# louissmit/VBNN

Measured on AMD Instinct MI355X. Metric: VBLinear fwd+bwd samples/sec, higher is better.
Workload: dtype bf16; 1 GPU; 784-4096-4096-10 VBLinear MLP, batch 4096 per GPU, LRT, S=1; mode=lrt, global_batch=4096, parallelism=dp1, warmup_steps_run=260, backward_order=every updateGradInput, then the accGradParameters from the first layer up, launch=one stream launch per kernel

## Files before the change

### include/vbnn_hip.h

```cpp
#ifndef VBNN_HIP_H
#define VBNN_HIP_H

#include <stddef.h>
#include <stdint.h>

#ifdef __cplusplus
extern "C" {
#endif
#if defined(__GNUC__)
#pragma GCC visibility push(default)
#endif

#define VBNN_ABI_VERSION 6
#define VBNN_KPAD 64

enum { VBNN_OK = 0, VBNN_ERR_INVALID = 1, VBNN_ERR_HIP = 2, VBNN_ERR_NOMEM = 3, VBNN_ERR_UNSUPPORTED = 4 };
enum { VBNN_F32 = 0, VBNN_BF16 = 1 };
enum { VBNN_PACK_COPY = 0, VBNN_PACK_EXP = 1, VBNN_PACK_SQUARE = 2, VBNN_PACK_MUL = 3,
       VBNN_PACK_RELU = 4, VBNN_PACK_RELU_SQUARE = 5 };

typedef struct vbnn_ctx vbnn_ctx;

int vbnn_abi_version(void);
const char* vbnn_last_error(void);
// ... 110 lines not shown
    void* g_prev; void* gv_prev; int64_t ld_gp;
    void* gT_prev; void* gvT_prev; int64_t ld_gpT;
    const void* w; const void* w2; int64_t ld_w;
} vbnn_dx_args;

int vbnn_grad_input(vbnn_ctx* ctx, int dtype, const vbnn_dx_args* a);

typedef struct vbnn_dw_args {
    const void* xT;
    const void* x2T;
    const void* gT;
    const void* gvT;
    int64_t ld_n;
    int64_t N, I, O;
    float scale;
    int accumulate;
    float* gradWeight;
    float* gradSum;
    uint64_t seed; uint32_t layer; uint32_t draw;
    const float* lvars;
    float* grad_mu; float* grad_lv;
    const float* means; const double* stats; float B; float S; float kl_scale;
    float* gradBias;
    const void* x; const void* x2; const void* g; const void* gv; int64_t ld_x; int64_t ld_g;
    const void* mu_s; const void* var_s; int64_t ld_w;
    int part;
    const uint32_t* draw_dev;
} vbnn_dw_args;

int vbnn_acc_grad_parameters(vbnn_ctx* ctx, int dtype, const vbnn_dw_args* a);

int vbnn_backward_pair(vbnn_ctx* ctx, int dtype, const vbnn_dx_args* dx, const vbnn_dw_args* dw);

int vbnn_acc_grad_bias(vbnn_ctx* ctx, int dtype, const void* g, int64_t ld_g, int64_t N, int64_t O,
                       float scale, int accumulate, float* gradBias);

int vbnn_prep_layer(vbnn_ctx* ctx, int dtype, const float* means, const float* lvars, int64_t O, int64_t I,
                    void* mu_s, void* var_s, int64_t ld_w, void* muT_s, void* varT_s, int64_t ld_wT,
                    double* stats);

typedef struct vbnn_prep_desc {
    const float* means; const float* lvars; int64_t O, I;
    void* mu_s; void* var_s; int64_t ld_w;
    void* muT_s; void* varT_s; int64_t ld_wT;
    double* stats;
} vbnn_prep_desc;
typedef struct vbnn_pack_desc {
    const float* src; int64_t rows, cols, ld_src;
    void* dst; int64_t ld_dst; void* dstT; int64_t ld_dstT;
} vbnn_pack_desc;
int vbnn_prepare(vbnn_ctx* ctx, int dtype, int n_layers, const vbnn_prep_desc* layers, const vbnn_pack_desc* extra);


int vbnn_compute_mugrads(vbnn_ctx* ctx, const float* means, const double* stats, float B, float S,
                         float* gradWeight, float* lcg, int64_t W);
int vbnn_compute_vargrads(vbnn_ctx* ctx, const float* lvars, const float* vars, const float* stdv,
                          const double* stats, float B, float S, float* gradSum, float* lcg, int64_t W);

int vbnn_calc_lc(vbnn_ctx* ctx, const float* means, const float* lvars, const float* vars, const float* mu_sqe,
                 const double* stats, float B, float* lc_elem, double* lc_sum_dev, int64_t W);

int vbnn_pack_input(vbnn_ctx* ctx, int dtype, const float* src, int64_t ld_src, int64_t N, int64_t I, void* x_s,
                    void* x2_s, int64_t ld_x, void* xT_s, void* x2T_s, int64_t ld_xT, int64_t rows_per_draw);


int vbnn_adam_step(vbnn_ctx* ctx, float* x, const float* grad, const float* grad2, float* m, float* v, int64_t n,
// ... 361 lines not shown
```

### vbnn_amd/_lib.py

```python
import ctypes as C
import os
import subprocess

_HERE = os.path.dirname(os.path.abspath(__file__))
LIB_PATH = os.environ.get("VBNN_HIP_LIB") or os.path.join(_HERE, "lib", "libvbnn_hip.so")
CSRC = os.path.join(_HERE, "csrc")

OK = 0
F32, BF16 = 0, 1
PACK_COPY, PACK_EXP, PACK_SQUARE, PACK_MUL, PACK_RELU, PACK_RELU_SQUARE = range(6)
KPAD = 64
STREAM_EPS, STREAM_ZETA, STREAM_INIT, STREAM_DATA, STREAM_HEINIT = 1, 2, 3, 4, 5

_vp, _i64, _u64, _u32, _f, _i = C.c_void_p, C.c_int64, C.c_uint64, C.c_uint32, C.c_float, C.c_int


class VbnnError(RuntimeError):
    pass


class FwdArgs(C.Structure):
    _fields_ = [("w", _vp), ("w2", _vp), ("x", _vp), ("x2", _vp), ("ld_w", _i64), ("ld_x", _i64),
                ("N", _i64), ("I", _i64), ("O", _i64), ("bias", _vp),
                ("seed", _u64), ("layer", _u32), ("draw", _u32), ("row0", _i64),
                ("y", _vp), ("ld_y", _i64), ("r", _vp), ("ld_r", _i64), ("r_packed", _i), ("relu", _i),
                ("h", _vp), ("h2", _vp), ("ld_h", _i64), ("hT", _vp), ("h2T", _vp), ("ld_hT", _i64), ("rows_per_draw", _i64),
                ("draw_dev", _vp), ("head_w3", _vp), ("head_ld_w", _i64), ("head_C", _i64), ("head_slots", _vp)]


class DxArgs(C.Structure):
    _fields_ = [("wT", _vp), ("w2T", _vp), ("g", _vp), ("gv", _vp), ("ld_wT", _i64), ("ld_g", _i64),
                ("N", _i64), ("I", _i64), ("O", _i64), ("x", _vp), ("ld_x", _i64),
                ("gx", _vp), ("ld_gx", _i64), ("relu_mask", _i), ("r_prev", _vp), ("ld_r_prev", _i64), ("r_prev_packed", _i),
                ("g_prev", _vp), ("gv_prev", _vp), ("ld_gp", _i64),
                ("gT_prev", _vp), ("gvT_prev", _vp), ("ld_gpT", _i64),
                ("w", _vp), ("w2", _vp), ("ld_w", _i64)]


class PrepDesc(C.Structure):
    _fields_ = [("means", _vp), ("lvars", _vp), ("O", _i64), ("I", _i64), ("mu_s", _vp), ("var_s", _vp), ("ld_w", _i64),
                ("muT_s", _vp), ("varT_s", _vp), ("ld_wT", _i64), ("stats", _vp)]

# ... 155 lines not shown

_SIGS = {
    "vbnn_abi_version": ([], _i),
    "vbnn_last_error": ([], C.c_char_p),
    "vbnn_debug_set": ([_i, _i], _i),
    "vbnn_debug_get": ([_i], _i),
    "vbnn_kmajor_supported": ([_i64, _i64, _i64], _i),
    "vbnn_kmajor_supported_dw": ([_i64, _i64, _i64, _i], _i),
    "vbnn_ctx_kmajor_supported": ([_vp, _i64, _i64, _i64], _i),
    "vbnn_ctx_kmajor_supported_dw": ([_vp, _i64, _i64, _i64, _i], _i),
    "vbnn_ctx_create": ([_i, _vp, C.POINTER(_vp)], _i),
    "vbnn_ctx_create_cu_budget": ([_i, _i, C.POINTER(_vp)], _i),
    "vbnn_ctx_stream": ([_vp, C.POINTER(_vp), C.POINTER(_i)], _i),
    "vbnn_ctx_destroy": ([_vp], _i),
    "vbnn_ctx_set_stream": ([_vp, _vp], _i),
    "vbnn_sync": ([_vp], _i),
    "vbnn_buf_alloc": ([_vp, C.c_size_t, C.POINTER(_vp)], _i),
    "vbnn_buf_free": ([_vp, _vp], _i),
    "vbnn_buf_zero": ([_vp, _vp, C.c_size_t], _i),
    "vbnn_buf_upload": ([_vp, _vp, _vp, C.c_size_t], _i),
    "vbnn_buf_download": ([_vp, _vp, _vp, C.c_size_t], _i),
    "vbnn_fill_normal": ([_vp, _vp, _i64, _i64, _i64, _u64, _u32, _u32, _u32, _i64, _f], _i),
    "vbnn_fill_normal_hw": ([_vp, _vp, _i64, _i64, _i64, _u64, _u32, _u32, _u32, _i64, _f], _i),
    "vbnn_box_muller_forms": ([_vp, _vp, _vp, _vp, _vp, _i64], _i),
    "vbnn_compute_prior": ([_vp, _vp, _vp, _i64, _vp, _vp, _vp, _vp], _i),
    "vbnn_wn_sample": ([_vp, _vp, _vp, _vp, _vp, _vp, _i64, _i64, _u64, _u32, _u32], _i),
    "vbnn_pack": ([_vp, _i, _i, _vp, _vp, _i64, _i64, _i64, _vp, _i64, _vp, _i64], _i),
    "vbnn_forward": ([_vp, _i, C.POINTER(FwdArgs)], _i),
    "vbnn_forward_head_slots": ([_vp, _i, _i64, _i64, _i64, _i64], _i),
    "vbnn_head_forward_slots": ([_vp, _vp, _i64, _vp, _vp, _i64, _i64, _f, _vp, _vp, _vp, _i, _vp, _vp, _i64], _i),
    "vbnn_grad_input": ([_vp, _i, C.POINTER(DxArgs)], _i),
    "vbnn_acc_grad_parameters": ([_vp, _i, C.POINTER(DwArgs)], _i),
    "vbnn_backward_pair": ([_vp, _i, C.POINTER(DxArgs), C.POINTER(DwArgs)], _i),
    "vbnn_head_forward_backward": ([_vp, _i, C.POINTER(HeadArgs)], _i),
    "vbnn_head_predict": ([_vp, _i, C.POINTER(PredictArgs)], _i),
    "vbnn_predict_moments": ([_vp, C.POINTER(MomentsArgs)], _i),
    "vbnn_acc_grad_bias": ([_vp, _i, _vp, _i64, _i64, _i64, _f, _i, _vp], _i),
    "vbnn_prep_layer": ([_vp, _i, _vp, _vp, _i64, _i64, _vp, _vp, _i64, _vp, _vp, _i64, _vp], _i),
    "vbnn_compute_mugrads": ([_vp, _vp, _vp, _f, _f, _vp, _vp, _i64], _i),
    "vbnn_compute_vargrads": ([_vp, _vp, _vp, _vp, _vp, _f, _f, _vp, _vp, _i64], _i),
    "vbnn_calc_lc": ([_vp, _vp, _vp, _vp, _vp, _vp, _f, _vp, _vp, _i64], _i),
    "vbnn_pack_input": ([_vp, _i, _vp, _i64, _i64, _i64, _vp, _vp, _i64, _vp, _vp, _i64, _i64], _i),
    "vbnn_adam_step": ([_vp, _vp, _vp, _vp, _vp, _vp, _i64, _f, _f, _f, _f, _f, _i64, _vp], _i),
    "vbnn_sgd_step": ([_vp, _vp, _vp, _i64, _f], _i),
    "vbnn_update": ([_vp, _i, _i, _vp, _vp], _i),
    "vbnn_prepare_masked": ([_vp, _i, _i, _vp, _vp, _vp], _i),
    "vbnn_update_masked": ([_vp, _i, _i, _vp, _vp, _vp], _i),
    "vbnn_calc_lc_masked": ([_vp, _vp, _vp, _vp, _vp, _f, _vp, _vp, _i64], _i),
    "vbnn_comm_unique_id": ([_vp], _i),
    "vbnn_comm_create": ([_vp, _i, _i, _vp, C.POINTER(_vp)], _i),
    "vbnn_comm_destroy": ([_vp], _i),
    "vbnn_comm_info": ([_vp, C.POINTER(_i), C.POINTER(_i), C.POINTER(_i)], _i),
    "vbnn_allreduce_grads": ([_vp, _vp, _i64], _i),
    "vbnn_comm_finish": ([_vp], _i),
    "vbnn_allreduce_grads_bf16": ([_vp, _vp, _i64], _i),
    "vbnn_cast_grads": ([_vp, _i, _vp, _vp, _i64], _i),
    "vbnn_comm_allgather_u64": ([_vp, _vp, _vp], _i),
    "vbnn_stats_combine": ([_vp, _i, _i, _vp, _vp], _i),
    "vbnn_transpose_packed": ([_vp, _i, _vp, _i64, _i64, _i64, _vp, _i64], _i),
    "vbnn_comm_reduce_scatter": ([_vp, _vp, _i64], _i),
    "vbnn_comm_all_gather": ([_vp, _vp, _i64], _i),
    "vbnn_p2p_reduce_scatter": ([_vp, C.c_size_t, _i64], _i),
    "vbnn_p2p_all_gather": ([_vp, C.c_size_t, _i64], _i),
    "vbnn_p2p_create": ([_vp, _i, _i, C.c_size_t, C.POINTER(_vp), C.POINTER(_vp), _vp], _i),
    "vbnn_p2p_connect": ([_vp, _vp], _i),
    "vbnn_p2p_allreduce": ([_vp, C.c_size_t, _i64], _i),
# ... 91 lines not shown
```

### vbnn_amd/csrc/gemm.hip

```cpp
#include "gemm_dispatch.h"

extern "C" int vbnn_debug_set(int key, int value) {
    if (key == VBNN_DEBUG_GEMM_KERNEL && value >= 0 && value <= 3) { g_force_kernel = value; return VBNN_OK; }
    if (key == VBNN_DEBUG_V2_SCHEDULE && (value == -1 || value == 0 || value == 2 || value == 4)) { g_v2_sched = value; return VBNN_OK; }
    if (key == VBNN_DEBUG_V2_TILE && (value == 0 || value == 64 || value == 128 || value == 256)) { g_v2_tile = value; return VBNN_OK; }
    if (key == VBNN_DEBUG_V3_MIN_K && value >= 64) { g_v3_min_k = value; return VBNN_OK; }
    if (key == VBNN_DEBUG_V2_PSPLIT && value >= -1 && value <= 1) { g_v2_psplit = value; return VBNN_OK; }
    if (key == VBNN_DEBUG_KMAJOR && value >= 0 && value <= 2) { g_kmajor = value; return VBNN_OK; }
    if (key == VBNN_DEBUG_V3_SPLIT && value >= -1 && value <= 1) { g_v3_split = value; return VBNN_OK; }
    if (key == VBNN_DEBUG_V0 && (value == 0 || value == 1)) { g_v0 = value; return VBNN_OK; }
    if (key == VBNN_DEBUG_HEAD_BACKWARD && value >= -1 && value <= 1) { g_head_stream = value; return VBNN_OK; }
    if (key == VBNN_DEBUG_V3_FOLD_SERIAL && (value == 0 || value == 1)) { g_v3_fold_serial = value; return VBNN_OK; }
    vbnn_set_error("vbnn_debug_set: unknown key %d / value %d", key, value);
    return VBNN_ERR_INVALID;
}
extern "C" int vbnn_debug_get(int key) {
    if (key == VBNN_DEBUG_LAST_HEAD_FORM) return g_last_head_form;
    if (key == VBNN_DEBUG_LAST_GEMM_FORM) return g_last_gemm_form;
    return -1;
}

extern "C" int vbnn_kmajor_supported(int64_t M, int64_t N, int64_t K) { return kmajor_selected(M, N, K) ? 1 : 0; }
extern "C" int vbnn_ctx_kmajor_supported(vbnn_ctx* ctx, int64_t M, int64_t N, int64_t K) {
    vbnn_cu_scope plan(ctx);
    return kmajor_selected(M, N, K) ? 1 : 0;
}
extern "C" int vbnn_kmajor_supported_dw(int64_t I, int64_t O, int64_t N, int bias_row) {
    if (!bias_row && kmajor_selected(I, O, N)) return 1;
    if (I % 4 == 0 && kmajor_dw_v3_split_selected(I + (bias_row ? 1 : 0), O, N)) return 2;
    return kmajor_dw_v2_selected(I + (bias_row ? 1 : 0), O, N) ? 1 : 0;
}
extern "C" int vbnn_ctx_kmajor_supported_dw(vbnn_ctx* ctx, int64_t I, int64_t O, int64_t N, int bias_row) {
    vbnn_cu_scope plan(ctx);
    return vbnn_kmajor_supported_dw(I, O, N, bias_row);
}

extern "C" int vbnn_backward_pair(vbnn_ctx* ctx, int dtype, const vbnn_dx_args* dx, const vbnn_dw_args* dw) {
    VBNN_API_BEGIN
    vbnn_cu_scope plan(ctx);
    int chk = check_dx_args(ctx, dx);
    if (chk != VBNN_OK) return chk;
    chk = check_dw_args(ctx, dtype, dw);
    if (chk != VBNN_OK) return chk;
    VBNN_REQUIRE(dx->N == dw->N && dx->I == dw->I && dx->O == dw->O, "the two argument blocks describe one layer");
    if (dtype == VBNN_F32 && !dx->wT && dx->w && !dw->xT && dw->x && dw->g && dw->part == 0 && g_force_kernel == 0) {
        const bool dual = dx->gv != nullptr;
        const bool dw_dual = dw->gv != nullptr;
        if (dual == dw_dual && (!dual || (dx->w2 && !dw->x2))) {
            const EpiDx<float> ea = make_dx_epi<float>(dx);
            const EpiDw eb = make_dw_epi<float>(dw);
            const int M2 = (int)dw->I + (dw->gradBias ? 1 : 0);
// ... 19 lines not shown
```

### vbnn_amd/csrc/gemm_v3.h

```cpp
#pragma once
#include "gemm_v2.h"

constexpr int V3_BM = 256, V3_BN = 256;
constexpr int V3_APART = 128 * 128;
constexpr int V3_BTILE = 256 * 128;
constexpr int V3_LDS = 4 * V3_APART + 3 * V3_BTILE;

inline int g_v3_min_k = 704;
inline int g_v3_fold_serial = 0;
template <class Epi, class = void> struct v3_fold_pipe { static constexpr int value = 0; };
template <class Epi> struct v3_fold_pipe<Epi, std::void_t<decltype(Epi::FOLD_PIPE)>> { static constexpr int value = Epi::FOLD_PIPE; };

#ifndef V3_ST
#define V3_ST(k) do { } while (0)
#endif


template <bool DUAL, bool AK, bool BK, class Epi, bool SPLIT = false, bool HM = false, int PIPE = v3_fold_pipe<Epi>::value>
__global__ __launch_bounds__(512, 2) void gemm_nt_v3(const bf16_t* __restrict__ A, const bf16_t* __restrict__ A2, int64_t lda,
                                                     const bf16_t* __restrict__ B, const bf16_t* __restrict__ B2, int64_t ldb,
                                                     int M, int N, int nk, int tiles_m, int tiles_n, Epi epi_in) {
    static_assert(!(SPLIT && DUAL), "the split form computes one GEMM of the pair per workgroup");
    static_assert(SPLIT == HM && (!HM || (AK && BK)), "the pair-split launch is the half-height K-major form");
    extern __shared__ __attribute__((aligned(16))) unsigned char lds[];
    V3_ST(0);
    const int tid = threadIdx.x;
    const int lane = tid & 63;
    const int wave = __builtin_amdgcn_readfirstlane(tid >> 6);
    if (wave >= 4) __builtin_amdgcn_s_setprio(1);
    const int wr = wave >> 2, wc = wave & 3;
    Epi epi = epi_in;

    const int nblk = tiles_m * tiles_n * (SPLIT ? 2 : 1);
    int bid = blockIdx.x;
    {
        const int q = nblk >> 3, r = nblk & 7, xcd = bid & 7, idx = bid >> 3;
        bid = (xcd < r ? xcd * (q + 1) : r * (q + 1) + (xcd - r) * q) + idx;
    }
    if (SPLIT) {
        const int ntile = tiles_m * tiles_n;
        const int part = bid / ntile;
        bid -= part * ntile;
        epi.set_part(1 + part);
        if (part) { A = A2; B = B2; }
    }
    int tm, tn;
    {
        constexpr int GM = HM ? 8 : 4, GN = HM ? 4 : 8;
        const int per_band = GM * tiles_n;
        const int band = bid / per_band;
        const int in_band = bid - band * per_band;
        const int band_rows = min(GM, tiles_m - band * GM);
        const int full = band_rows * GN;
        const int grp = in_band / full;
        const int in_grp = in_band - grp * full;
        const int grp_cols = min(GN, tiles_n - grp * GN);
        tm = min(band * GM + in_grp / grp_cols, tiles_m - 1);
        tn = grp * GN + in_grp % grp_cols;
    }
    const int m0 = tm * (HM ? V3_BM / 2 : V3_BM), n0 = tn * V3_BN;

    int a_off[2][2], b_off[4];
    auto hk = [](int kr) { return (kr & 3) | (((kr >> 3) & 1) << 2); };
#pragma unroll
    for (int P = 0; P < 2; ++P)
#pragma unroll
        for (int d = 0; d < 2; ++d) {
// ... 694 lines not shown
                if (DUAL) epi.apply_folded(wm0, wn0 + 4 * p, eln, r1[p], r2[p], pre[b], t1, t2);
                else epi.apply_fast(wm0, wn0 + 4 * p, eln, r1[p], f32x4{0.f, 0.f, 0.f, 0.f}, pre[b], t1, t2);
                if (any_t) {
                    const int nl = 4 * p + q4;
                    const int col = ((nl >> 3) ^ (c16 & 3)) * 8 + (nl & 7);
#pragma unroll
                    for (int j = 0; j < 4; ++j) {
                        tl1[(4 * c16 + j) * TQ + col] = Elt<ET>::to(t1[j]);
                        tl2[(4 * c16 + j) * TQ + col] = Elt<ET>::to(t2[j]);
                    }
                }
                __builtin_amdgcn_sched_barrier(0);
            }
        }
        if (any_t) {
            const int64_t ldt = epi.t_ld();
            const unsigned lo = (unsigned)((lane >> 2) * (int)ldt + 8 * (lane & 3));
#pragma unroll
            for (int pp = 0; pp < 4; ++pp) {
                const int ml = 16 * pp + (lane >> 2);
                const int64_t ub = (int64_t)(wm0 + 16 * pp) * ldt + wn0;
                if (tp1)
                    *reinterpret_cast<bf16x8*>(tp1 + ub + lo) =
                        *reinterpret_cast<const bf16x8*>(tl1 + ml * TQ + 8 * ((lane & 3) ^ ((ml >> 2) & 3)));
                if (tp2)
                    *reinterpret_cast<bf16x8*>(tp2 + ub + lo) =
                        *reinterpret_cast<const bf16x8*>(tl2 + ml * TQ + 8 * ((lane & 3) ^ ((ml >> 2) & 3)));
            }
        }
    });
    V3_ST(4);
}

template <class Epi>
static inline bool gemm_v3_possible(int64_t M, int64_t N, int64_t K, int64_t lda, int64_t ldb, bool ak, bool bk, const Epi& epi) {
    Epi e = epi;
    const bool t_ok = (!e.t1_ptr() && !e.t2_ptr()) ||
                      ((e.t_ld() % 8 == 0) && ((((uintptr_t)e.t1_ptr() | (uintptr_t)e.t2_ptr()) & 15u) == 0));
    const bool a_ok = ak ? (K % V2_BK == 0 && lda % 8 == 0 && lda >= M && K * lda < (1ll << 30)) : M * lda < (1ll << 30);
    const bool b_ok = bk ? (K % V2_BK == 0 && ldb % 8 == 0 && ldb >= N && K * ldb < (1ll << 30)) : N * ldb < (1ll << 30);
    return (M % V3_BM == 0) && (N % V3_BN == 0) && a_ok && b_ok && epi.fast_ok() && epi.v3_ok() && t_ok && M * e.t_ld() < (1ll << 31);
}
static inline bool gemm_v3_shape_ok(int64_t M, int64_t N, int64_t K) {
    if (M % V3_BM || N % V3_BN || K < g_v3_min_k) return false;
    const int64_t cus = vbnn_cu_count();
    const int64_t t3 = (M / V3_BM) * (N / V3_BN), t2 = 2 * t3;
    if (4 * t3 < 3 * cus) return false;
    const int64_t r3 = (t3 + cus - 1) / cus, r2 = (t2 + cus - 1) / cus;
    return 185 * r3 <= 100 * r2;
}
template <class Epi>
static inline bool gemm_v3_eligible(int64_t M, int64_t N, int64_t K, int64_t lda, int64_t ldb, bool ak, bool bk, const Epi& epi) {
    if (!gemm_v3_possible(M, N, K, lda, ldb, ak, bk, epi) || K < g_v3_min_k) return false;
    const int64_t cus = vbnn_cu_count();
    const int64_t t3 = (M / V3_BM) * (N / V3_BN), t2 = 2 * t3;
    if (4 * t3 < 3 * cus) return false;
    const int64_t r3 = (t3 + cus - 1) / cus, r2 = (t2 + cus - 1) / cus;
    return 185 * r3 <= 100 * r2;
}

template <typename T, bool DUAL, bool AK, bool BK, class Epi>
static int launch_gemm_v3(vbnn_ctx* ctx, const T* A, const T* A2, int64_t lda, const T* B, const T* B2, int64_t ldb, int M, int N,
                          int K, const Epi& epi) {
    if constexpr (sizeof(T) != 2) {
        vbnn_set_error("gemm_v3 is bf16 only");
        return VBNN_ERR_UNSUPPORTED;
// ... 4 lines not shown
        }
        const int nk = (K + V2_BK - 1) / V2_BK;
        if ((!AK && lda < (int64_t)nk * V2_BK) || (!BK && ldb < (int64_t)nk * V2_BK)) {
            vbnn_set_error("packed leading dimension too small for K=%d", K);
            return VBNN_ERR_INVALID;
        }
        if (!gemm_v3_possible(M, N, K, lda, ldb, AK, BK, epi)) { vbnn_set_error("gemm_v3: shape / outputs outside its fast path"); return VBNN_ERR_UNSUPPORTED; }
        const int tiles_m = (M + V3_BM - 1) / V3_BM, tiles_n = (N + V3_BN - 1) / V3_BN;
        const void* kern = (const void*)gemm_nt_v3<DUAL, AK, BK, Epi>;
        int form = 0;
        if constexpr (DUAL && v3_fold_pipe<Epi>::value != 0) {
            if (g_v3_fold_serial) { kern = (const void*)gemm_nt_v3<DUAL, AK, BK, Epi, false, false, 0>; form = 1; }
        }
        static vbnn_per_device_flag configured_on[2];
        bool& configured = configured_on[form][ctx->device];
        if (!configured) {
            hipError_t e = hipFuncSetAttribute(kern, hipFuncAttributeMaxDynamicSharedMemorySize, V3_LDS);
            if (e != hipSuccess) { vbnn_set_error("hipFuncSetAttribute: %s", hipGetErrorString(e)); return VBNN_ERR_HIP; }
            configured = true;
        }
        const bf16_t* a = (const bf16_t*)A; const bf16_t* a2 = (const bf16_t*)A2;
        const bf16_t* b = (const bf16_t*)B; const bf16_t* b2 = (const bf16_t*)B2;
        int nk_ = nk, M_ = M, N_ = N, tm_ = tiles_m, tn_ = tiles_n;
        int64_t lda_ = lda, ldb_ = ldb;
        Epi epi_ = epi;
        void* args[] = {&a, &a2, &lda_, &b, &b2, &ldb_, &M_, &N_, &nk_, &tm_, &tn_, &epi_};
        vbnn_note_gemm_form<T>(VBNN_GEMM_KERNEL_V3, 0, 0, DUAL, false, AK, BK, 0, false, form == 1, epi);
        hipError_t e = hipLaunchKernel(kern, dim3(tiles_m * tiles_n), dim3(512), args, V3_LDS, ctx->stream);
        if (e != hipSuccess) { vbnn_set_error("launch of gemm_nt_v3 failed: %s", hipGetErrorString(e)); return VBNN_ERR_HIP; }
        return vbnn_check_launch("gemm_nt_v3");
    }
}

inline int g_v3_split = -1;
static inline bool gemm_v3_split_shape_ok(int64_t M, int64_t N, int64_t K) {
    if (g_v3_split == 0 || N % V3_BN || K % V2_BK) return false;
    if (g_v3_split == 1) return true;
    const int64_t tiles = ((M + V3_BM - 1) / V3_BM) * (N / V3_BN);
    const int64_t blocks = ((M + V3_BM / 2 - 1) / (V3_BM / 2)) * (N / V3_BN) * 2;
    const int64_t cus = vbnn_cu_count();
    return tiles * 16 <= 5 * cus && tiles * 16 >= 3 * cus && K >= 2048 && blocks <= cus && blocks * 8 >= 5 * cus;
}
static inline int64_t gemm_v3_split_lda(int64_t M) { return (M + V3_BM - 1) / V3_BM * V3_BM; }

template <typename T, class Epi>
static int launch_gemm_v3_split(vbnn_ctx* ctx, const T* A, const T* A2, int64_t lda, const T* B, const T* B2, int64_t ldb, int M, int N,
                                int K, const Epi& epi) {
    if constexpr (sizeof(T) != 2 || !Epi::SPLITTABLE || !Epi::EDGE_FAST) {
        return VBNN_ERR_UNSUPPORTED;
    } else {
        Epi e0 = epi;
        if (!A || !A2 || !B || !B2 || !gemm_v3_split_shape_ok(M, N, K) || !epi.fast_ok() || e0.t1_ptr() || e0.t2_ptr() ||
            (((uintptr_t)A | (uintptr_t)B | (uintptr_t)A2 | (uintptr_t)B2) & 15u) != 0 || lda % 8 || ldb % 8 ||
            lda < gemm_v3_split_lda(M) || ldb < N || (int64_t)K * lda >= (1ll << 30) || (int64_t)K * ldb >= (1ll << 30))
            return VBNN_ERR_UNSUPPORTED;
        const int tiles_n = N / V3_BN;
        const int tiles_m = (M + V3_BM / 2 - 1) / (V3_BM / 2);
        const void* kern = (const void*)gemm_nt_v3<false, true, true, Epi, true, true>;
        static vbnn_per_device_flag configured_on;
        bool& configured = configured_on[ctx->device];
        if (!configured) {
            hipError_t e = hipFuncSetAttribute(kern, hipFuncAttributeMaxDynamicSharedMemorySize, V3_LDS);
            if (e != hipSuccess) { vbnn_set_error("hipFuncSetAttribute: %s", hipGetErrorString(e)); return VBNN_ERR_HIP; }
            configured = true;
        }
        const bf16_t* a = (const bf16_t*)A; const bf16_t* a2 = (const bf16_t*)A2;
// ... 12 lines not shown
```

### vbnn_amd/engine.py

```python
import contextlib
import ctypes as C
import math
import os

import torch

from . import _lib as L
from . import partition
from .nn import Context, _DT, _Packed, _VB, _ordered, _p, fill_normal
from .predictive import (LabelPredictResult, PredictResult, QuantilePredictResult, RegressionPredictResult,
                         _Predictive)
from .calibration import CalibrationResult, SelectiveResult, _Calibration
from .pruning import PruneResult, SparsePruneResult, UnitPruneResult, _Pruning
from .checkpoint import CheckpointError, _Checkpoint, digest


_NULL_CM = contextlib.nullcontext()


class _View:

    def __init__(self, t):
        self.t, self.ld = t, t.stride(0)

# ... 40 lines not shown
        ts = self.ctx.torch_stream
        if ts is None:
            return _NULL_CM
        cur = torch.cuda.current_stream(self.device)
        if cur != ts:
            ts.wait_stream(cur)
        return torch.cuda.stream(ts)

    def join(self):
        ts = self.ctx.torch_stream
        if ts is not None:
            cur = torch.cuda.current_stream(self.device)
            if cur != ts:
                cur.wait_stream(ts)

    def _build(self, opt, world_size, rank, process_group, force_reduce):
        self.dtype = opt.get("dtype", "bf16")
        self.code, self.tdt = _DT[self.dtype]
        self.mode = opt.get("mode", "lrt")
        assert self.mode in ("wn", "lrt")
        self.seed = int(opt.get("seed", 3))
        self.world, self.rank, self.pg = world_size, rank, process_group
        self.reduce = world_size > 1 or force_reduce
        self._exchange = None
        self.exchange_dtype = str(opt.get("exchange_dtype", "f32"))
        assert self.exchange_dtype in ("f32", "bf16")
        self._stage, self._staged = None, []
        self.exchange_mode = str(opt.get("exchange_mode", os.environ.get("VBNN_EXCHANGE_MODE", "")) or "allreduce")
        assert self.exchange_mode in ("allreduce", "sharded")
        self.sharded = self.reduce and self.exchange_mode == "sharded"
        self._params_stale = False
        self._dx_first_opt = opt.get("dx_first", None)
        self.fuse_kl = bool(opt.get("fuse_kl", True))
        self.criterion = opt.get("criterion", "nll")
        assert self.criterion in ("nll", "mse", "gauss", "bce")
        self.logvar_clamp = tuple(float(v) for v in opt.get("logvar_clamp", (-20.0, 20.0)))
        if self.criterion == "gauss":
            if int(opt["n_classes"]) % 2:
                raise ValueError(f"criterion = 'gauss': the final Linear holds D means and D log variances (n_classes = "
                                 f"{opt['n_classes']} is odd)")
            if not (len(self.logvar_clamp) == 2 and self.logvar_clamp[0] <= self.logvar_clamp[1]):
                raise ValueError(f"opt.logvar_clamp = {self.logvar_clamp}: (s_min, s_max) with s_min <= s_max")
        self.kl_from_shadows = self.dtype == "bf16" and bool(opt.get("kl_from_shadows", True))
        self.kl_in_update = bool(opt.get("kl_in_update", self.kl_from_shadows and self.fuse_kl and self.mode == "lrt"))
        if self.sharded:
            assert self.fuse_kl and self.mode == "lrt" and self.exchange_dtype == "f32" and not opt.get("overlap", False), \
                "exchange_mode = sharded: the fused LRT engine, fp32 sums, one compute stream"
            assert self.dtype == "bf16" and self.kl_from_shadows, "exchange_mode = sharded: the bf16 configuration (operand shadows)"
            self.kl_in_update = True
        assert not self.kl_in_update or (self.fuse_kl and self.mode == "lrt"), "kl_in_update: the fused LRT engine"
        self.overlap = bool(opt.get("overlap", False))
        self.head_step = bool(opt.get("head_step", True))
        if self.overlap:
            self._side = torch.cuda.Stream(device=self.device)
            self.ctx2 = Context(self.device.index or 0, stream=self._side)
        self.B, self.S = float(opt.get("B", 1e6)), float(opt.get("S", 1))
        hidden = list(opt["hidden"])
        sizes = [opt["input_size"]] + hidden
        self.n_classes = opt["n_classes"]
        self.sizes = sizes
        weights = [sizes[i] * sizes[i + 1] for i in range(len(sizes) - 1)]
        self.dx_first = bool(self._dx_first_opt) if self._dx_first_opt is not None else (2 * min(weights) <= max(weights))
        dev = self.device
        f32 = dict(dtype=torch.float32, device=dev)
        el = opt.get("early_lv", None)
        if el is None:
            el = [(world_size > 1 or force_reduce) and self.mode == "lrt" and bool(opt.get("fuse_kl", True)) and
                  sizes[i] * sizes[i + 1] >= (1 << 22) for i in range(len(hidden))]
        elif isinstance(el, bool):
            el = [el and self.mode == "lrt"] * len(hidden)
        self.early_lv = list(el)
        lay, fin, n_g, self._bucket_ranges = partition.arena_layout(sizes, self.n_classes, self.early_lv)
        self._lay = lay
        self.exchange_kind = str(opt.get("exchange", os.environ.get("VBNN_EXCHANGE", "")) or "")
        n_layers = len(hidden)
        self._plan = partition.sharded_plan(lay, world_size) if self.sharded else None
        arena_extra = None
        if self.reduce and self.exchange_kind == "p2p":
            assert self.exchange_dtype == "f32", "the p2p exchange sums fp32 arenas"
            from .comm import P2PExchange
            n_arena = (n_g + 3) // 4 * 4
            if self.sharded:
                n_arena += sum(2 * _Packed.floats(sizes[i + 1], sizes[i], self.tdt) for i in range(n_layers)) + 8 * world_size * n_layers
            self._exchange = P2PExchange(self.ctx, rank, world_size, n_arena, process_group)
            self.grads = self._exchange.arena[:n_g]
            arena_extra = self._exchange.arena[(n_g + 3) // 4 * 4:]
        else:
            self.grads = torch.zeros(n_g, **f32)

        def carve(n_floats):
            nonlocal arena_extra
            if arena_extra is None:
                return None
            piece, arena_extra = arena_extra[:n_floats], arena_extra[n_floats:]
            return piece
# ... 193 lines not shown

    def _w3_pack_desc(self):
        return L.PackDesc(src=_p(self.weight3), rows=self.n_classes, cols=self.sizes[-1], ld_src=self.sizes[-1],
                          dst=self.w3_s.ptr, ld_dst=self.w3_s.ld, dstT=self.w3T_s.ptr, ld_dstT=self.w3T_s.ld)

    def _lrt(self):
        return self.mode == "lrt" and not self._map

    probe = None

    def _probed(self, name, li):
        if self.probe is None or (self.probe[0] != li and self.probe[0] != "all"):
            return contextlib.nullcontext()
        if self.probe[0] == "all":
            name = f"{name}[{li}]"
        eng = self

        class _Bracket:
            def __enter__(self_inner):
                self_inner.e0 = torch.cuda.Event(enable_timing=True)
                self_inner.e1 = torch.cuda.Event(enable_timing=True)
                self_inner.e0.record()

            def __exit__(self_inner, *exc):
                self_inner.e1.record()
                eng.probe[1].setdefault(name, []).append((self_inner.e0, self_inner.e1))
                return False
        return _Bracket()

    def _probed_part(self, name, li):
        if self.probe is None or self.probe[0] != "all" or not self._early(self.vb[li], self._lrt()):
            return _NULL_CM
        return self._probed(name, li)

    @_ordered
    def clamp_to_map(self):
        self._map = True
        if self.mode == "wn":
            lib = L.lib()
            for v in self.vb:
                L.check(lib.vbnn_pack(self.ctx.h, self.code, L.PACK_COPY, _p(v.means), None, v.I, v.O, v.I,
                                      v.mu_s.ptr, v.mu_s.ld, v.muT_s.ptr if v.muT_s else None,
                                      v.muT_s.ld if v.muT_s else 0))

    def test(self, inputs, targets):
        N = inputs.shape[0]
        self.prepare()
        draws = 1 if self.opt.get("quicktest") else int(self.opt["testSamples"])
        err = acc = 0.0
        for _ in range(draws):
            self._first = True
            if self.opt.get("quicktest"):
                self.clamp_to_map()
            else:
                self.sample()
            self.run(inputs, targets, backward=False)
            loss, correct = self.loss_and_accuracy()
            err += loss * self.world
            acc += 100.0 * correct / (N * (self.n_classes if self.criterion == "bce" else 1))
        return err / draws, acc / draws

    @_ordered
    def sample(self, by=1):
        self.draw += by
        self._map = False
        if self.device_draw:
# ... 214 lines not shown
                                                        inv_n, _p(self.logits), _p(self.out), _p(self.g_logits), accumulate,
                                                        _p(self._acc), _p(self._corr), self._rpd))
                else:
                    L.check(lib.vbnn_head_forward(ctx, code, self.h_s.ptr, self.h_s.ld, self.w3_s.ptr, self.w3_s.ld,
                                                  _p(self.bias3), _p(targets), N, H, Cn, inv_n, _p(self.logits), _p(self.out),
                                                  _p(self.g_logits), accumulate, _p(self._acc), _p(self._corr), self._rpd))
                if not backward:
                    self._first = False
                    return
                L.check(lib.vbnn_head_backward(ctx, code, self.h_s.ptr, self.h_s.ld, self.w3_s.ptr, self.w3_s.ld,
                                               _p(self.g_logits), N, H, Cn, accumulate, _p(self.gradWeight3),
                                               _p(self.gradBias3), _p(vl.gradBias), 1, _p(vl.r) if lrt else None, vl.O, 1,
                                               vl.g_s.ptr,
                                               vl.gv_s.ptr if lrt else None, vl.g_s.ld, vl.gT_s.ptr if vl.gT_s else None,
                                               vl.gvT_s.ptr if (lrt and vl.gvT_s) else None, vl.gT_s.ld if vl.gT_s else 0))
        else:
            if self._rpd:
                targets = targets.repeat(self._draws) if targets.dim() == 1 else targets.repeat(self._draws, 1)
            self._generic_head(N, targets, inv_n, accumulate, backward)
            if not backward:
                self._first = False
                return
        if self.f32_direct and not self.overlap:
            for li in range(nl - 1, -1, -1):
                v = self.vb[li]
                d = self._dw_args(li, N, accumulate)
                with self._probed("accGradParameters", li):
                    if li > 0:
                        L.check(lib.vbnn_backward_pair(ctx, code, C.byref(self._dx_args(li, N)), C.byref(d)))
                    else:
                        L.check(lib.vbnn_acc_grad_parameters(ctx, code, C.byref(d)))
                if not (fused_head and li == nl - 1) and not v.bias_from_dw:
                    L.check(lib.vbnn_acc_grad_bias(ctx, code, v.g_s.ptr, v.g_s.ld, N, v.O, 1.0, accumulate, _p(v.gradBias)))
        elif self.dx_first and not self.reduce and not self.overlap:
            for li in range(nl - 1, 0, -1):
                with self._probed("updateGradInput", li):
                    L.check(lib.vbnn_grad_input(ctx, code, C.byref(self._dx_args(li, N))))
            for li in range(nl):
                v = self.vb[li]
                d = self._dw_args(li, N, accumulate)
                with self._probed("accGradParameters", li):
                    L.check(lib.vbnn_acc_grad_parameters(ctx, code, C.byref(d)))
                if not (fused_head and li == nl - 1) and not v.bias_from_dw:
                    L.check(lib.vbnn_acc_grad_bias(ctx, code, v.g_s.ptr, v.g_s.ld, N, v.O, 1.0, accumulate, _p(v.gradBias)))
        elif not self.overlap:
            for li in range(nl - 1, -1, -1):
                v = self.vb[li]
                d = self._dw_args(li, N, accumulate)
                with self._probed("accGradParameters", li):
                    if self._early(v, lrt):
                        d.part = 2
                        with self._probed_part("accGradParameters.lv", li):
                            L.check(lib.vbnn_acc_grad_parameters(ctx, code, C.byref(d)))
                        if self.sharded:
                            self._scatter(li, ("lv",))
                        else:
                            self._reduce(v.msg_early)
                        d.part = 1
                    with self._probed_part("accGradParameters.mu", li):
                        L.check(lib.vbnn_acc_grad_parameters(ctx, code, C.byref(d)))
                if not (fused_head and li == nl - 1) and not v.bias_from_dw:
                    L.check(lib.vbnn_acc_grad_bias(ctx, code, v.g_s.ptr, v.g_s.ld, N, v.O, 1.0, accumulate, _p(v.gradBias)))
                if self.sharded:
                    self._scatter(li, ("mu", "small") if self._early(v, lrt) else ("lv", "mu", "small"))
                else:
                    self._reduce(v.msg_late if self._early(v, lrt) else (self.bucket_tail if li == nl - 1 else v.bucket))
# ... 306 lines not shown
```

Baseline: 5.572 million samples/s.

## Chain each layer's grad-input and grad-weight GEMMs into one persistent launch

Adds a combined kernel that runs the dX GEMM and the dW GEMM of one hidden layer inside a single launch. Each workgroup computes its tile of the first GEMM, passes an LDS barrier, then computes its tile of the second. The engine enables this by default for bf16 when the dx-first heuristic holds. This reorders the backward pass to per-layer dx/dw pairs. The aim is to cut one kernel launch per layer and the idle tail between the two GEMMs. The cost is a grid sized to the larger of the two GEMMs and a fused kernel that may use registers differently.

```diff
diff --git a/include/vbnn_hip.h b/include/vbnn_hip.h
--- a/include/vbnn_hip.h
+++ b/include/vbnn_hip.h
@@ -166,6 +166,12 @@
 
 int vbnn_backward_pair(vbnn_ctx* ctx, int dtype, const vbnn_dx_args* dx, const vbnn_dw_args* dw);
 
+#define VBNN_CHAIN_DX_FIRST 0
+#define VBNN_CHAIN_DW_FIRST 1
+#define VBNN_DEBUG_LAST_CHAINED 15
+#define VBNN_DEBUG_CHAIN_OFF 16
+int vbnn_backward_chain(vbnn_ctx* ctx, int dtype, const vbnn_dx_args* dx, const vbnn_dw_args* dw, int order);
+
 int vbnn_acc_grad_bias(vbnn_ctx* ctx, int dtype, const void* g, int64_t ld_g, int64_t N, int64_t O,
                        float scale, int accumulate, float* gradBias);
 
diff --git a/vbnn_amd/_lib.py b/vbnn_amd/_lib.py
--- a/vbnn_amd/_lib.py
+++ b/vbnn_amd/_lib.py
@@ -8,6 +8,8 @@
 
 OK = 0
 F32, BF16 = 0, 1
+CHAIN_DX_FIRST, CHAIN_DW_FIRST = 0, 1
+DEBUG_LAST_CHAINED, DEBUG_CHAIN_OFF = 15, 16
 PACK_COPY, PACK_EXP, PACK_SQUARE, PACK_MUL, PACK_RELU, PACK_RELU_SQUARE = range(6)
 KPAD = 64
 STREAM_EPS, STREAM_ZETA, STREAM_INIT, STREAM_DATA, STREAM_HEINIT = 1, 2, 3, 4, 5
@@ -229,6 +231,7 @@
     "vbnn_grad_input": ([_vp, _i, C.POINTER(DxArgs)], _i),
     "vbnn_acc_grad_parameters": ([_vp, _i, C.POINTER(DwArgs)], _i),
     "vbnn_backward_pair": ([_vp, _i, C.POINTER(DxArgs), C.POINTER(DwArgs)], _i),
+    "vbnn_backward_chain": ([_vp, _i, C.POINTER(DxArgs), C.POINTER(DwArgs), _i], _i),
     "vbnn_head_forward_backward": ([_vp, _i, C.POINTER(HeadArgs)], _i),
     "vbnn_head_predict": ([_vp, _i, C.POINTER(PredictArgs)], _i),
     "vbnn_predict_moments": ([_vp, C.POINTER(MomentsArgs)], _i),
diff --git a/vbnn_amd/csrc/gemm.hip b/vbnn_amd/csrc/gemm.hip
--- a/vbnn_amd/csrc/gemm.hip
+++ b/vbnn_amd/csrc/gemm.hip
@@ -11,12 +11,14 @@
     if (key == VBNN_DEBUG_V0 && (value == 0 || value == 1)) { g_v0 = value; return VBNN_OK; }
     if (key == VBNN_DEBUG_HEAD_BACKWARD && value >= -1 && value <= 1) { g_head_stream = value; return VBNN_OK; }
     if (key == VBNN_DEBUG_V3_FOLD_SERIAL && (value == 0 || value == 1)) { g_v3_fold_serial = value; return VBNN_OK; }
+    if (key == VBNN_DEBUG_CHAIN_OFF && (value == 0 || value == 1)) { g_v3_chain_off = value; return VBNN_OK; }
     vbnn_set_error("vbnn_debug_set: unknown key %d / value %d", key, value);
     return VBNN_ERR_INVALID;
 }
 extern "C" int vbnn_debug_get(int key) {
     if (key == VBNN_DEBUG_LAST_HEAD_FORM) return g_last_head_form;
     if (key == VBNN_DEBUG_LAST_GEMM_FORM) return g_last_gemm_form;
+    if (key == VBNN_DEBUG_LAST_CHAINED) return g_v3_last_chained;
     return -1;
 }
 
diff --git a/vbnn_amd/csrc/gemm_chain.hip b/vbnn_amd/csrc/gemm_chain.hip
--- /dev/null
+++ b/vbnn_amd/csrc/gemm_chain.hip
@@ -0,0 +1,54 @@
+#include "gemm_dispatch.h"
+
+static bool chain_dx_ok(const vbnn_dx_args* a, const EpiDx<bf16_t>& e) {
+    return a->gv && a->w && a->w2 && a->g && !a->gT_prev && !a->gvT_prev && kmajor_selected(a->I, a->N, a->O) &&
+           gemm_v3_possible(a->I, a->N, a->O, a->ld_w, a->ld_g, true, false, e);
+}
+static bool chain_dw_ok(const vbnn_dw_args* a, const EpiDw& e) {
+    if (a->part != 0 || a->accumulate != 0 || !e.lrt || a->gradBias || e.has_draw_dev()) return false;
+    if (!a->x || !a->x2 || !a->g || !a->gv) return false;
+    if (a->gT && a->gvT && g_kmajor) return false;
+    return kmajor_selected(a->I, a->O, a->N) && gemm_v3_possible(a->I, a->O, a->N, a->ld_x, a->ld_g, true, true, e);
+}
+
+extern "C" int vbnn_backward_chain(vbnn_ctx* ctx, int dtype, const vbnn_dx_args* dx, const vbnn_dw_args* dw, int order) {
+    VBNN_API_BEGIN
+    vbnn_cu_scope plan(ctx);
+    int chk = check_dx_args(ctx, dx);
+    if (chk != VBNN_OK) return chk;
+    chk = check_dw_args(ctx, dtype, dw);
+    if (chk != VBNN_OK) return chk;
+    VBNN_REQUIRE(dx->N == dw->N && dx->I == dw->I && dx->O == dw->O, "the two argument blocks describe one layer");
+    VBNN_REQUIRE(order == VBNN_CHAIN_DX_FIRST || order == VBNN_CHAIN_DW_FIRST, "order: VBNN_CHAIN_DX_FIRST or VBNN_CHAIN_DW_FIRST");
+    g_v3_last_chained = 0;
+    if (dtype == VBNN_BF16 && !g_v3_chain_off) {
+        const EpiDx<bf16_t> ex = make_dx_epi<bf16_t>(dx);
+        const EpiDw ew = make_dw_epi<bf16_t>(dw);
+        if (chain_dx_ok(dx, ex) && chain_dw_ok(dw, ew)) {
+            const bf16_t* w = (const bf16_t*)dx->w;  const bf16_t* w2 = (const bf16_t*)dx->w2;
+            const bf16_t* g = (const bf16_t*)dx->g;  const bf16_t* gv = (const bf16_t*)dx->gv;
+            const bf16_t* x = (const bf16_t*)dw->x;  const bf16_t* x2 = (const bf16_t*)dw->x2;
+            const bf16_t* h = (const bf16_t*)dw->g;  const bf16_t* hv = (const bf16_t*)dw->gv;
+            int st;
+            if (order == VBNN_CHAIN_DX_FIRST)
+                st = launch_gemm_v3_chain<bf16_t, true, false, EpiDx<bf16_t>, true, true, EpiDw>(
+                    ctx, w, w2, dx->ld_w, g, gv, dx->ld_g, (int)dx->I, (int)dx->N, (int)dx->O, ex,
+                    x, x2, dw->ld_x, h, hv, dw->ld_g, (int)dw->I, (int)dw->O, (int)dw->N, ew);
+            else
+                st = launch_gemm_v3_chain<bf16_t, true, true, EpiDw, true, false, EpiDx<bf16_t>>(
+                    ctx, x, x2, dw->ld_x, h, hv, dw->ld_g, (int)dw->I, (int)dw->O, (int)dw->N, ew,
+                    w, w2, dx->ld_w, g, gv, dx->ld_g, (int)dx->I, (int)dx->N, (int)dx->O, ex);
+            if (st == VBNN_OK) g_v3_last_chained = 1;
+            if (st != VBNN_ERR_UNSUPPORTED) return st;
+        }
+    }
+    if (order == VBNN_CHAIN_DX_FIRST) {
+        const int st = vbnn_grad_input(ctx, dtype, dx);
+        if (st != VBNN_OK) return st;
+        return vbnn_acc_grad_parameters(ctx, dtype, dw);
+    }
+    const int st = vbnn_acc_grad_parameters(ctx, dtype, dw);
+    if (st != VBNN_OK) return st;
+    return vbnn_grad_input(ctx, dtype, dx);
+    VBNN_API_END
+}
diff --git a/vbnn_amd/csrc/gemm_v3.h b/vbnn_amd/csrc/gemm_v3.h
--- a/vbnn_amd/csrc/gemm_v3.h
+++ b/vbnn_amd/csrc/gemm_v3.h
@@ -17,9 +17,9 @@
 
 
 template <bool DUAL, bool AK, bool BK, class Epi, bool SPLIT = false, bool HM = false, int PIPE = v3_fold_pipe<Epi>::value>
-__global__ __launch_bounds__(512, 2) void gemm_nt_v3(const bf16_t* __restrict__ A, const bf16_t* __restrict__ A2, int64_t lda,
-                                                     const bf16_t* __restrict__ B, const bf16_t* __restrict__ B2, int64_t ldb,
-                                                     int M, int N, int nk, int tiles_m, int tiles_n, Epi epi_in) {
+__device__ __forceinline__ void gemm_nt_v3_body(const int wg, const bf16_t* __restrict__ A, const bf16_t* __restrict__ A2, int64_t lda,
+                                                const bf16_t* __restrict__ B, const bf16_t* __restrict__ B2, int64_t ldb,
+                                                int M, int N, int nk, int tiles_m, int tiles_n, const Epi& epi_in) {
     static_assert(!(SPLIT && DUAL), "the split form computes one GEMM of the pair per workgroup");
     static_assert(SPLIT == HM && (!HM || (AK && BK)), "the pair-split launch is the half-height K-major form");
     extern __shared__ __attribute__((aligned(16))) unsigned char lds[];
@@ -32,7 +32,7 @@
     Epi epi = epi_in;
 
     const int nblk = tiles_m * tiles_n * (SPLIT ? 2 : 1);
-    int bid = blockIdx.x;
+    int bid = wg;
     {
         const int q = nblk >> 3, r = nblk & 7, xcd = bid & 7, idx = bid >> 3;
         bid = (xcd < r ? xcd * (q + 1) : r * (q + 1) + (xcd - r) * q) + idx;
@@ -793,6 +793,28 @@
     V3_ST(4);
 }
 
+template <bool DUAL, bool AK, bool BK, class Epi, bool SPLIT = false, bool HM = false, int PIPE = v3_fold_pipe<Epi>::value>
+__global__ __launch_bounds__(512, 2) void gemm_nt_v3(const bf16_t* __restrict__ A, const bf16_t* __restrict__ A2, int64_t lda,
+                                                     const bf16_t* __restrict__ B, const bf16_t* __restrict__ B2, int64_t ldb,
+                                                     int M, int N, int nk, int tiles_m, int tiles_n, Epi epi_in) {
+    gemm_nt_v3_body<DUAL, AK, BK, Epi, SPLIT, HM, PIPE>(blockIdx.x, A, A2, lda, B, B2, ldb, M, N, nk, tiles_m, tiles_n, epi_in);
+}
+
+struct v3_gemm_args {
+    const bf16_t* A; const bf16_t* A2; int64_t lda;
+    const bf16_t* B; const bf16_t* B2; int64_t ldb;
+    int M, N, nk, tiles_m, tiles_n;
+};
+template <bool AK1, bool BK1, class Epi1, bool AK2, bool BK2, class Epi2>
+__global__ __launch_bounds__(512, 2) void gemm_nt_v3_chain(v3_gemm_args g1, Epi1 e1, v3_gemm_args g2, Epi2 e2) {
+    const int wg = blockIdx.x;
+    if (wg < g1.tiles_m * g1.tiles_n)
+        gemm_nt_v3_body<true, AK1, BK1, Epi1>(wg, g1.A, g1.A2, g1.lda, g1.B, g1.B2, g1.ldb, g1.M, g1.N, g1.nk, g1.tiles_m, g1.tiles_n, e1);
+    v2_lds_barrier();
+    if (wg < g2.tiles_m * g2.tiles_n)
+        gemm_nt_v3_body<true, AK2, BK2, Epi2>(wg, g2.A, g2.A2, g2.lda, g2.B, g2.B2, g2.ldb, g2.M, g2.N, g2.nk, g2.tiles_m, g2.tiles_n, e2);
+}
+
 template <class Epi>
 static inline bool gemm_v3_possible(int64_t M, int64_t N, int64_t K, int64_t lda, int64_t ldb, bool ak, bool bk, const Epi& epi) {
     Epi e = epi;
@@ -863,6 +885,44 @@
     }
 }
 
+inline int g_v3_chain_off = 0;
+inline int g_v3_last_chained = 0;
+template <typename T, bool AK1, bool BK1, class Epi1, bool AK2, bool BK2, class Epi2>
+static int launch_gemm_v3_chain(vbnn_ctx* ctx, const T* A, const T* A2, int64_t lda, const T* B, const T* B2, int64_t ldb, int M, int N, int K,
+                                const Epi1& epi1, const T* C, const T* C2, int64_t ldc, const T* D, const T* D2, int64_t ldd, int P, int Q,
+                                int R, const Epi2& epi2) {
+    if constexpr (sizeof(T) != 2) {
+        return VBNN_ERR_UNSUPPORTED;
+    } else {
+        if ((((uintptr_t)A | (uintptr_t)B | (uintptr_t)A2 | (uintptr_t)B2 | (uintptr_t)C | (uintptr_t)D | (uintptr_t)C2 | (uintptr_t)D2) & 15u) != 0)
+            return VBNN_ERR_UNSUPPORTED;
+        const int nk1 = (K + V2_BK - 1) / V2_BK, nk2 = (R + V2_BK - 1) / V2_BK;
+        if ((!AK1 && lda < (int64_t)nk1 * V2_BK) || (!BK1 && ldb < (int64_t)nk1 * V2_BK) || (!AK2 && ldc < (int64_t)nk2 * V2_BK) ||
+            (!BK2 && ldd < (int64_t)nk2 * V2_BK))
+            return VBNN_ERR_UNSUPPORTED;
+        if (!gemm_v3_possible(M, N, K, lda, ldb, AK1, BK1, epi1) || !gemm_v3_possible(P, Q, R, ldc, ldd, AK2, BK2, epi2)) return VBNN_ERR_UNSUPPORTED;
+        const void* kern = (const void*)gemm_nt_v3_chain<AK1, BK1, Epi1, AK2, BK2, Epi2>;
+        static vbnn_per_device_flag configured_on;
+        bool& configured = configured_on[ctx->device];
+        if (!configured) {
+            hipError_t e = hipFuncSetAttribute(kern, hipFuncAttributeMaxDynamicSharedMemorySize, V3_LDS);
+            if (e != hipSuccess) { vbnn_set_error("hipFuncSetAttribute: %s", hipGetErrorString(e)); return VBNN_ERR_HIP; }
+            configured = true;
+        }
+        v3_gemm_args g1 = {(const bf16_t*)A, (const bf16_t*)A2, lda, (const bf16_t*)B, (const bf16_t*)B2, ldb, M, N, nk1, M / V3_BM, N / V3_BN};
+        v3_gemm_args g2 = {(const bf16_t*)C, (const bf16_t*)C2, ldc, (const bf16_t*)D, (const bf16_t*)D2, ldd, P, Q, nk2, P / V3_BM, Q / V3_BN};
+        Epi1 e1 = epi1;
+        Epi2 e2 = epi2;
+        void* args[] = {&g1, &e1, &g2, &e2};
+        const int n1 = g1.tiles_m * g1.tiles_n, n2 = g2.tiles_m * g2.tiles_n;
+        vbnn_note_gemm_form<T>(VBNN_GEMM_KERNEL_V3, 0, 0, true, false, AK1, BK1, 0, false, false, epi1);
+        vbnn_note_gemm_form<T>(VBNN_GEMM_KERNEL_V3, 0, 0, true, false, AK2, BK2, 0, false, false, epi2);
+        hipError_t e = hipLaunchKernel(kern, dim3(n1 > n2 ? n1 : n2), dim3(512), args, V3_LDS, ctx->stream);
+        if (e != hipSuccess) { vbnn_set_error("launch of gemm_nt_v3_chain failed: %s", hipGetErrorString(e)); return VBNN_ERR_HIP; }
+        return vbnn_check_launch("gemm_nt_v3_chain");
+    }
+}
+
 inline int g_v3_split = -1;
 static inline bool gemm_v3_split_shape_ok(int64_t M, int64_t N, int64_t K) {
     if (g_v3_split == 0 || N % V3_BN || K % V2_BK) return false;
diff --git a/vbnn_amd/engine.py b/vbnn_amd/engine.py
--- a/vbnn_amd/engine.py
+++ b/vbnn_amd/engine.py
@@ -96,6 +96,10 @@
         self._params_stale = False
         self._dx_first_opt = opt.get("dx_first", None)
         self.fuse_kl = bool(opt.get("fuse_kl", True))
+        cb = opt.get("chain_backward", os.environ.get("VBNN_CHAIN_BACKWARD"))
+        cb = "dx" if cb is True else ("" if cb in (False, "0", 0, "") else cb)
+        assert cb in (None, "", "dx", "dw"), "chain_backward: 'dx', 'dw' or off"
+        self._chain_opt = cb
         self.criterion = opt.get("criterion", "nll")
         assert self.criterion in ("nll", "mse", "gauss", "bce")
         self.logvar_clamp = tuple(float(v) for v in opt.get("logvar_clamp", (-20.0, 20.0)))
@@ -125,6 +129,8 @@
         self.sizes = sizes
         weights = [sizes[i] * sizes[i + 1] for i in range(len(sizes) - 1)]
         self.dx_first = bool(self._dx_first_opt) if self._dx_first_opt is not None else (2 * min(weights) <= max(weights))
+        self.chain_backward = "" if self.dtype != "bf16" else (self._chain_opt if self._chain_opt is not None else
+                                                                ("dx" if self.dx_first and self._dx_first_opt is None else ""))
         dev = self.device
         f32 = dict(dtype=torch.float32, device=dev)
         el = opt.get("early_lv", None)
@@ -384,6 +390,16 @@
         if self.probe is None or self.probe[0] != "all" or not self._early(self.vb[li], self._lrt()):
             return _NULL_CM
         return self._probed(name, li)
+
+    def _chain_as_two_probed(self, li, N, d, order):
+        lib, ctx, code = L.lib(), self.ctx.h, self.code
+        fams = ("updateGradInput", "accGradParameters") if order == L.CHAIN_DX_FIRST else ("accGradParameters", "updateGradInput")
+        for fam in fams:
+            with self._probed(fam, li):
+                if fam == "updateGradInput":
+                    L.check(lib.vbnn_grad_input(ctx, code, C.byref(self._dx_args(li, N))))
+                else:
+                    L.check(lib.vbnn_acc_grad_parameters(ctx, code, C.byref(d)))
 
     @_ordered
     def clamp_to_map(self):
@@ -664,6 +680,23 @@
                         L.check(lib.vbnn_acc_grad_parameters(ctx, code, C.byref(d)))
                 if not (fused_head and li == nl - 1) and not v.bias_from_dw:
                     L.check(lib.vbnn_acc_grad_bias(ctx, code, v.g_s.ptr, v.g_s.ld, N, v.O, 1.0, accumulate, _p(v.gradBias)))
+        elif self.chain_backward and not self.reduce and not self.overlap:
+            order = L.CHAIN_DW_FIRST if self.chain_backward == "dw" else L.CHAIN_DX_FIRST
+            for li in range(nl - 1, 0, -1):
+                v = self.vb[li]
+                d = self._dw_args(li, N, accumulate)
+                if self.probe is not None and self.probe[0] in (li, "all"):
+                    self._chain_as_two_probed(li, N, d, order)
+                else:
+                    L.check(lib.vbnn_backward_chain(ctx, code, C.byref(self._dx_args(li, N)), C.byref(d), order))
+                if not (fused_head and li == nl - 1) and not v.bias_from_dw:
+                    L.check(lib.vbnn_acc_grad_bias(ctx, code, v.g_s.ptr, v.g_s.ld, N, v.O, 1.0, accumulate, _p(v.gradBias)))
+            v = self.vb[0]
+            d = self._dw_args(0, N, accumulate)
+            with self._probed("accGradParameters", 0):
+                L.check(lib.vbnn_acc_grad_parameters(ctx, code, C.byref(d)))
+            if not (fused_head and nl == 1) and not v.bias_from_dw:
+                L.check(lib.vbnn_acc_grad_bias(ctx, code, v.g_s.ptr, v.g_s.ld, N, v.O, 1.0, accumulate, _p(v.gradBias)))
         elif self.dx_first and not self.reduce and not self.overlap:
             for li in range(nl - 1, 0, -1):
                 with self._probed("updateGradInput", li):
```

Result: faster. 5.674 million samples/s (median of 6 runs) (+1.8%).
